# skhu101/TDNN-F_NAS

Hardware: AMD Instinct MI355X
Metric: LF-MMI training frames/sec per node (SWBD 7q TDNN-F) (higher is better)
Workload: dtype f32

## Files before the change

tdnn-f_nas_amd/csrc/abi_tdnn.hip:

```cpp
#include <dlfcn.h>
#include <stdlib.h>
#include <string.h>

#include <string>

#include "common.h"
#include "gemm_f32.h"
#include "planes_gemm.h"

namespace tdnnf {

static thread_local std::string g_last_error;

void set_error(const char *fmt, ...) {
  char buf[1024];
  va_list ap;
  va_start(ap, fmt);
  vsnprintf(buf, sizeof(buf), fmt, ap);
  va_end(ap);
  g_last_error = buf;
}
int hip_status(hipError_t e, const char *what) {
  set_error("HIP error %d (%s) in %s", (int)e, hipGetErrorString(e), what);
  return TDNNF_EHIP;
// ... 4 lines not shown
  return o;
}

namespace {
typedef int (*roctx_push_t)(const char *);
typedef int (*roctx_pop_t)();
roctx_push_t g_roctx_push = nullptr;
roctx_pop_t g_roctx_pop = nullptr;
bool roctx_ready() {
  static const bool ok = [] {
    const char *e = getenv("TDNNF_ROCTX");
    if (e && atoi(e) == 0) return false;
    for (const char *lib : {"librocprofiler-sdk-roctx.so", "librocprofiler-sdk-roctx.so.1", "libroctx64.so", "libroctx64.so.4"}) {
      void *h = dlopen(lib, RTLD_NOW | RTLD_GLOBAL);
      if (!h) continue;
      g_roctx_push = (roctx_push_t)dlsym(h, "roctxRangePushA");
      g_roctx_pop = (roctx_pop_t)dlsym(h, "roctxRangePop");
      if (g_roctx_push && g_roctx_pop) return true;
    }
    return false;
  }();
  return ok;
}
}
TraceRange::TraceRange(const char *name) : on(roctx_ready()) {
  if (on) g_roctx_push(name);
}
TraceRange::~TraceRange() {
  if (on) g_roctx_pop();
}

bool tdnn_rows_ok(const tdnnf_tdnn_indexes *ix, int rows_in, int N) {
  if (!ix || ix->num_offsets < 1 || ix->num_offsets > TDNNF_MAX_OFFSETS || ix->row_stride < 1) return false;
  for (int i = 0; i < ix->num_offsets; i++) {
    const long long need = (long long)ix->row_offsets[i] + (long long)ix->row_stride * N - (ix->row_stride - 1);
    if (ix->row_offsets[i] < 0 || (N > 0 && rows_in < need)) return false;
  }
  return true;
}

}

using namespace tdnnf;

extern "C" {

const char *tdnnf_last_error(void) { return g_last_error.c_str(); }
int tdnnf_abi_version(void) { return 1; }

static int *option_slot(const char *name) {
  Options &o = options();
  if (!name) return nullptr;
  const struct { const char *n; int *p; } table[] = {{"ng_grouped", &o.ng_grouped}, {"ng_fuse", &o.ng_fuse}, {"ng_early_in", &o.ng_early_in},
                                                     {"wgrad_stream", &o.wgrad_stream}, {"gemm_ring", &o.gemm_ring}, {"planes", &o.planes}, {"den_split", &o.den_split}, {"phase_events", &o.phase_events}, {"wgrad_lag", &o.wgrad_lag}, {"ng_bk", &o.ng_bk}, {"ng_valu", &o.ng_valu}, {"ng_pform", &o.ng_pform}, {"planes_group", &o.planes_group}, {"xent_behind_den", &o.xent_behind_den}, {"ng_early_fork", &o.ng_early_fork}, {"ng_diag_skip", &o.ng_diag_skip}, {"wgrad_small", &o.wgrad_small}, {"splitk_per_cu", &o.splitk_per_cu}, {"gemm_alt_taps", &o.gemm_alt_taps}, {"reverse_passes", &o.reverse_passes}, {"splitk_partial_round", &o.splitk_partial_round}, {"wgrad_on_caller", &o.wgrad_on_caller}, {"den_mw_test_abort", &o.den_mw_test_abort}, {"planes_check_bound", &o.planes_check_bound}, {"den_gamma_pairs", &o.den_gamma_pairs}, {"num_form", &o.num_form}, {"num_frontier_cap", &o.num_frontier_cap}, {"gemm_arith_test", &o.gemm_arith_test}};
  for (auto &e : table)
    if (strcmp(e.n, name) == 0) return e.p;
  return nullptr;
}
int tdnnf_set_option(const char *name, int value) {
  int *p = option_slot(name);
  TDNNF_REQUIRE(p, "set_option: unknown option '%s' (ng_grouped, ng_fuse, ng_early_in, wgrad_stream, gemm_ring, planes, den_split)", name ? name : "(null)");
  *p = value;
  return TDNNF_OK;
}
int tdnnf_get_option(const char *name, int *value) {
  int *p = option_slot(name);
  TDNNF_REQUIRE(p && value, "get_option: unknown option '%s'", name ? name : "(null)");
  *value = *p;
  return TDNNF_OK;
}

}

namespace tdnnf {
int tdnn_propagate_impl(const tdnnf_tdnn_indexes *ix, const tdnnf_mat *in, const float *W, int ldw, int Do, int Di,
                        const float *bias, const float *eff_coef, int init_mode, int relu, tdnnf_mat *out, tdnnf_stream stream,
                        float *colstats, int *colstats_rows) {
  TDNNF_REQUIRE(mat_ok(in) && mat_ok(out) && W, "tdnn_propagate: bad matrices");
  TDNNF_REQUIRE(Do > 0 && Di > 0 && in->cols == Di && out->cols == Do, "tdnn_propagate: dims: in.cols=%d Di=%d out.cols=%d Do=%d",
                in ? in->cols : -1, Di, out ? out->cols : -1, Do);
  TDNNF_REQUIRE(tdnn_rows_ok(ix, in->rows, out->rows), "tdnn_propagate: input has too few rows for the time offsets");
  TDNNF_REQUIRE(ldw >= ix->num_offsets * Di, "tdnn_propagate: ldw < K*Di");
  TDNNF_REQUIRE(init_mode >= 0 && init_mode <= 2 && (init_mode != 1 || bias), "tdnn_propagate: init_mode 1 needs a bias");
  RowsGemmArgs a;
  memset(&a, 0, sizeof(a));
  a.A = in->data;
  a.lda = (long long)in->stride * ix->row_stride;
  a.B = W;
  a.ldb = ldw;
  a.C = out->data;
  a.ldc = out->stride;
  a.M = out->rows;
  a.N = Do;
  a.bias = bias;
  a.coef = eff_coef;
  a.init_mode = init_mode;
  a.relu = relu;
  a.colstats = colstats;
  a.colstats_rows = colstats_rows;
  a.nseg = ix->num_offsets;
  for (int i = 0; i < a.nseg; i++) {
    a.seg[i].a_off = (long long)ix->row_offsets[i] * in->stride;
    a.seg[i].b_off = (long long)i * Di;
    a.seg[i].klen = Di;
    a.seg[i].m_lo = 0;
    a.seg[i].m_hi = out->rows;
  }
// ... 201 lines not shown
```

tdnn-f_nas_amd/csrc/common.h:

```cpp
#pragma once
#include <hip/hip_runtime.h>
#include <stdarg.h>
#include <stdio.h>

#include "tdnnf_hip.h"

namespace tdnnf {

struct MatView {
  float *data;
  int rows, cols, stride;
};
inline MatView view(const tdnnf_mat *m) { return MatView{m->data, m->rows, m->cols, m->stride}; }

void set_error(const char *fmt, ...);
int hip_status(hipError_t e, const char *what);

inline bool mat_ok(const tdnnf_mat *m) {
  return m && m->rows >= 0 && m->cols >= 0 && m->stride >= m->cols && (m->data || m->rows * m->cols == 0);
}
inline bool same_dim(const tdnnf_mat *a, const tdnnf_mat *b) { return a->rows == b->rows && a->cols == b->cols; }

inline bool vec4_ok(const MatView &m) {
  return (reinterpret_cast<uintptr_t>(m.data) & 15) == 0 && m.stride % 4 == 0 && m.cols % 4 == 0;
}

#define TDNNF_REQUIRE(cond, ...)            \
  do {                                      \
    if (!(cond)) {                          \
      ::tdnnf::set_error(__VA_ARGS__);      \
      return TDNNF_EINVAL;                  \
    }                                       \
  } while (0)

#define TDNNF_HIP(expr)                                         \
  do {                                                          \
    hipError_t e__ = (expr);                                    \
    if (e__ != hipSuccess) return ::tdnnf::hip_status(e__, #expr); \
  } while (0)

#define TDNNF_LAUNCH_CHECK() TDNNF_HIP(hipGetLastError())

struct Options {
  int ng_grouped = 1;
  int ng_fuse = 1;
  int ng_early_in = 1;
  int wgrad_stream = -1;
  int gemm_ring = 1;
  int planes = 1;
  int den_mw_test_abort = 0;
  int planes_group = 1;
  int planes_check_bound = 0;
  int wgrad_lag = 3;
  int wgrad_on_caller = 0;
  int splitk_partial_round = 1;
  int reverse_passes = 0;
  int gemm_alt_taps = 1;
  int splitk_per_cu = 2;
  int wgrad_small = 0;
  int ng_bk = 0;
  int ng_early_fork = 1;
  int xent_behind_den = -1;
  int ng_pform = 1;
  int ng_valu = 0;
  int ng_diag_skip = 0;
  int phase_events = 0;
  int den_split = -1;
  int num_form = 0;
  int gemm_arith_test = 0;
  int num_frontier_cap = 0;
  int den_gamma_pairs = 0;
};
Options &options();

struct TraceRange {
  explicit TraceRange(const char *name);
  ~TraceRange();
  bool on;
};

__host__ __device__ inline float floor_keep_nan(float x, float f) { return x < f ? f : x; }

inline int grid_for(long long work, int block, int cap = 2048) {
  long long g = (work + block - 1) / block;
  if (g > cap) g = cap;
  if (g < 1) g = 1;
  return (int)g;
}
#ifdef __HIPCC__
template <class T>
struct as_given { typedef T type; };
template <class... P>
__attribute__((visibility("hidden"))) inline hipError_t launch_vec_or_scalar(bool vec, int rows, int cols, void (*k4)(P...), void (*k1)(P...), hipStream_t s, typename as_given<P>::type... args) {
  const long long work = (long long)rows * (vec ? cols / 4 : cols);
  void (*k)(P...) = vec ? k4 : k1;
  hipLaunchKernelGGL(k, dim3(grid_for(work, 256)), dim3(256), 0, s, args...);
  return hipGetLastError();
}
#endif

inline unsigned long long tdnnf_decision(unsigned long long step, unsigned long long k) {
  unsigned long long z = step * 0x9E3779B97F4A7C15ULL + k * 0xBF58476D1CE4E5B9ULL + 0x94D049BB133111EBULL;
  z = (z ^ (z >> 30)) * 0xBF58476D1CE4E5B9ULL;
  z = (z ^ (z >> 27)) * 0x94D049BB133111EBULL;
  return (z ^ (z >> 31)) >> 8;
}

bool log_softmax_propagate_with_aux(const tdnnf_mat *in, tdnnf_mat *out, tdnnf_mat *aux, float aux_scale, hipStream_t s);
float chain_supervision_weight(const tdnnf_supervision *sp);
size_t chain_split_region_bytes(const tdnnf_den_graph *g, int B, int T);
int chain_den(const tdnnf_den_graph *g, const tdnnf_supervision *sp, const tdnnf_mat *y, float leaky, tdnnf_mat *deriv, void *ws, hipStream_t s,
              bool beside_other_work = false, hipStream_t caller_aux = nullptr, hipEvent_t ev_recursions = nullptr, bool *ev_recorded = nullptr);
int chain_num_recursion(const tdnnf_supervision *sp, const tdnnf_den_graph *g, const tdnnf_mat *y, void *ws, hipStream_t s);
int chain_num_xent(const tdnnf_den_graph *g, const tdnnf_supervision *sp, const tdnnf_mat *y, const tdnnf_mat *xent_output, float xent_regularize,
                   tdnnf_mat *xent_deriv, void *ws, hipStream_t s, bool xent_deriv_initialised = false);
int chain_num(const tdnnf_den_graph *g, const tdnnf_supervision *sp, const tdnnf_mat *y, const tdnnf_mat *xent_output,
              float xent_regularize, tdnnf_mat *xent_deriv, void *ws, hipStream_t s, bool xent_deriv_initialised = false);
int chain_finish(const tdnnf_den_graph *g, const tdnnf_supervision *sp, const tdnnf_mat *y, float l2_regularize, double *results,
                 tdnnf_mat *deriv, tdnnf_mat *xent_deriv, void *ws, hipStream_t s);
int chain_objf_den(const tdnnf_den_graph *g, const tdnnf_supervision *sp, const tdnnf_mat *y, float leaky, void *ws, hipStream_t s);
int chain_objf_num_recursion(const tdnnf_supervision *sp, const tdnnf_den_graph *g, const tdnnf_mat *y, void *ws, hipStream_t s);
int chain_objf_num_xent(const tdnnf_den_graph *g, const tdnnf_supervision *sp, const tdnnf_mat *y, const tdnnf_mat *xent_output, void *ws, hipStream_t s);
int chain_objf_finish(const tdnnf_den_graph *g, const tdnnf_supervision *sp, const tdnnf_mat *y, float l2_regularize, double *results, void *ws, hipStream_t s);
// ... 14 lines not shown
```

tdnn-f_nas_amd/csrc/launch_forms.h:

```cpp
#pragma once
#include <atomic>

namespace tdnnf {

enum RowsForm {
  kFormPlain,
  kFormRing,
  kFormSplitK,
  kFormPartialS2,
  kFormPartialS8 = kFormPartialS2 + 6,
  kFormMainSplitTail,
  kFormMainPlainTail,
  kFormSumsqPlain,
  kFormSumsqSplitK,
  kFormPost,
  kFormGrouped,
  kRowsForms
};
constexpr int kRowsTiles = 9, kRowsAriths = 3;

template <int WM, int WN, int TM, int TN, int BK>
constexpr int rows_tile_index() {
  constexpr int BM = WM * TM * 32, BN = WN * TN * 32;
  constexpr int t = (BM == 128 && BN == 32 && BK == 32) ? 0 : (BM == 128 && BN == 32 && BK == 64) ? 1 : (BM == 128 && BN == 64 && BK == 32) ? 2
                  : (BM == 128 && BN == 96 && BK == 16) ? 3 : (BM == 128 && BN == 96 && BK == 32) ? 4 : (BM == 128 && BN == 160 && BK == 16) ? 5
                  : (BM == 64 && BN == 128 && BK == 16) ? 6 : (BM == 128 && BN == 128 && BK == 16) ? 7 : (BM == 128 && BN == 128 && BK == 32) ? 8 : -1;
  static_assert(t >= 0, "a rows GEMM tile without a counter: add it here and to kRowsTileNames (launch_forms.hip)");
  return t;
}
constexpr int rows_form_index(int tile, int arith, int form) { return (tile * kRowsAriths + arith) * kRowsForms + form; }

enum {
  kPlanesPlain = kRowsTiles * kRowsAriths * kRowsForms,
  kPlanesMainSplitTail,
  kPlanesMainPlainTail,
  kWgradFirst,
  kWgradPlanes = kWgradFirst + 5 * kRowsAriths,
  kWgradLastSlabs,
  kRowsLastSlices,
  kRowsVec4Launches,
  kRowsScalarLaunches,
  kPlanesAltChunked,
  kLaunchFormCounters
};

std::atomic<long long> *launch_form_counters();
inline void count_form(int index) { launch_form_counters()[index].fetch_add(1, std::memory_order_relaxed); }
inline void note_rows_slices(int ksplit) { launch_form_counters()[kRowsLastSlices].store(ksplit, std::memory_order_relaxed); }
inline void note_wgrad_slabs(int splits) { launch_form_counters()[kWgradLastSlabs].store(splits, std::memory_order_relaxed); }

}
```

tdnn-f_nas_amd/csrc/launch_forms.hip:

```cpp
#include "launch_forms.h"

#include <stdio.h>

#include "common.h"

namespace tdnnf {

std::atomic<long long> *launch_form_counters() {
  static std::atomic<long long> counters[kLaunchFormCounters];
  return counters;
}

namespace {
const char *const kRowsTileNames[kRowsTiles] = {"128x32k32", "128x32k64", "128x64k32", "128x96k16", "128x96k32", "128x160k16", "64x128k16", "128x128k16", "128x128k32"};
const char *const kArithNames[kRowsAriths] = {"f32", "bf16x3", "bf16x6"};
const char *const kRowsFormNames[kRowsForms] = {"plain", "ring", "splitk", "partial_s2", "partial_s3", "partial_s4", "partial_s5", "partial_s6", "partial_s7", "partial_s8",
                                                "main_split_tail", "main_plain_tail", "sumsq_plain", "sumsq_splitk", "post", "grouped"};
const char *const kWgradTileNames[5] = {"128x128", "160x128", "128x160", "32x128", "64x64"};
}

}

using namespace tdnnf;

extern "C" {

const char *tdnnf_gemm_launch_form_name(int index) {
  static thread_local char buf[64];
  if (index < 0 || index >= kLaunchFormCounters) return nullptr;
  if (index < kPlanesPlain) {
    const int form = index % kRowsForms, arith = (index / kRowsForms) % kRowsAriths, tile = index / (kRowsForms * kRowsAriths);
    snprintf(buf, sizeof(buf), "rows.%s.%s.%s", kRowsTileNames[tile], kArithNames[arith], kRowsFormNames[form]);
  } else if (index == kPlanesPlain) {
    snprintf(buf, sizeof(buf), "planes.plain");
  } else if (index == kPlanesMainSplitTail) {
    snprintf(buf, sizeof(buf), "planes.main_split_tail");
  } else if (index == kPlanesMainPlainTail) {
    snprintf(buf, sizeof(buf), "planes.main_plain_tail");
  } else if (index < kWgradPlanes) {
    const int i = index - kWgradFirst;
    snprintf(buf, sizeof(buf), "wgrad.%s.%s", kWgradTileNames[i / kRowsAriths], kArithNames[i % kRowsAriths]);
  } else if (index == kWgradPlanes) {
    snprintf(buf, sizeof(buf), "wgrad.planes");
  } else if (index == kWgradLastSlabs) {
    snprintf(buf, sizeof(buf), "wgrad.last_slabs");
  } else if (index == kRowsLastSlices) {
    snprintf(buf, sizeof(buf), "rows.last_slices");
  } else if (index == kRowsVec4Launches) {
    snprintf(buf, sizeof(buf), "rows.launches_vec4");
  } else if (index == kRowsScalarLaunches) {
    snprintf(buf, sizeof(buf), "rows.launches_scalar");
  } else {
    snprintf(buf, sizeof(buf), "planes.alt_chunked");
  }
  return buf;
}

int tdnnf_gemm_launch_forms(long long *counts, int capacity, int reset) {
  std::atomic<long long> *c = launch_form_counters();
  for (int i = 0; i < kLaunchFormCounters; i++) {
    if (counts && i < capacity) counts[i] = c[i].load(std::memory_order_relaxed);
    if (reset) c[i].store(0, std::memory_order_relaxed);
  }
  return kLaunchFormCounters;
}

}
```

tdnn-f_nas_amd/csrc/ng_stats.hip:

```cpp
#include <string.h>

#include <algorithm>

#include "gemm_f32.h"
#include "ng.h"
#include "ng_kernels.h"

namespace tdnnf {
namespace {

size_t part_bytes(int N) { return ((size_t)rows_gemm_sumsq_blocks(N) * sizeof(double) + 63) & ~(size_t)63; }
size_t stats_ws_bytes(int Rp, int Di, int K, int N) {
  return part_bytes(N) + std::max(std::max(wgrad_workspace_bytes(Rp, Rp, 1, N), wgrad_workspace_bytes(Rp, Di, K, N)), ng_pform_ws_bytes(Rp, Di, K, N));
}

constexpr int kPformSpanCap = 4096;
struct TapSpan {
  int lo, hi;
};
TapSpan tap_span(const tdnnf_tdnn_indexes &ix) {
  TapSpan t{ix.row_offsets[0], ix.row_offsets[0]};
  for (int i = 1; i < ix.num_offsets; i++) {
    t.lo = std::min(t.lo, ix.row_offsets[i]);
    t.hi = std::max(t.hi, ix.row_offsets[i]);
// ... 26 lines not shown
  for (int i = 0; i < K; i++) tp.o[i] = in.ix.row_offsets[i] - sp.lo;
  const int M = N + (sp.hi - sp.lo);
  float *WP = (float *)ws;
  float *P = WP + (((size_t)K * Rp * Di + 63) & ~(size_t)63);
  double *psum = (double *)(P + (((size_t)M * K * Rp + 63) & ~(size_t)63));
  hipLaunchKernelGGL(stack_taps_kernel, dim3(grid_for((long long)K * Rp * Di, 256)), dim3(256), 0, s, W, Rp, ldw, Di, K, WP);
  TDNNF_HIP(rows_gemm_1seg(in.x.data + (size_t)sp.lo * in.x.stride, in.x.stride, WP, Di, true, P, K * Rp, M, K * Rp, Di, 2, nullptr, psum, s));
  hipLaunchKernelGGL(pform_combine_kernel, dim3(N / 128), dim3(256), 0, s, P, K * Rp, tp, Rp, bias, H, N, psum, part,
                     rows_gemm_sumsq_blocks(N));
  TDNNF_HIP(hipGetLastError());
  return TDNNF_OK;
}

RowsGemmArgs ng_pass_gemm_args(const float *W, int ldw, int Rp, const float *bias, const NgInput &in, float *H, int ldh, double *part) {
  const int N = in.N, K = in.ix.num_offsets, Di = in.Di;
  RowsGemmArgs a;
  memset(&a, 0, sizeof(a));
  a.A = in.x.data; a.lda = (long long)in.x.stride * in.ix.row_stride; a.B = W; a.ldb = ldw; a.C = H; a.ldc = ldh; a.M = N; a.N = Rp;
  a.bias = bias;
  a.init_mode = bias ? 1 : 2;
  a.coef = in.eff;
  a.sumsq = part;
  a.nseg = K;
  for (int i = 0; i < K; i++) {
    a.seg[i].a_off = (long long)in.ix.row_offsets[i] * in.x.stride;
    a.seg[i].b_off = (long long)i * Di;
    a.seg[i].klen = Di;
    a.seg[i].m_lo = 0;
    a.seg[i].m_hi = N;
  }
  return a;
}
NgRowdotArgs ng_pass_rowdot_args(const float *WT, int Rp, const float *bias, const NgInput &in, float *H, int ldh, double *part, int part_cap) {
  const int K = in.ix.num_offsets;
  NgRowdotArgs v;
  memset(&v, 0, sizeof(v));
  v.X = in.x.data; v.ldx = in.x.stride; v.row_stride = in.ix.row_stride; v.nseg = K; v.Di = in.Di; v.eff = in.eff; v.WT = WT; v.Rp = Rp;
  v.bias = bias; v.H = H; v.ldh = ldh; v.N = in.N; v.part = part; v.part_cap = part_cap;
  for (int i = 0; i < K; i++) v.seg_off[i] = (long long)in.ix.row_offsets[i] * in.x.stride;
  return v;
}

namespace {

const float *ones_column(const tdnnf_ng *ng, const NgInput &in) { return in.ones ? ng->wlast : nullptr; }

int stats_after_h(tdnnf_ng *ng, const NgInput &in, const float *H, void *wg_ws, size_t wg_bytes, bool upd, hipStream_t s) {
  const int N = in.N, K = in.ix.num_offsets, Di = in.Di, Rp = ng->Rp, Dp = ng->Dp, D = ng->D;
  ng->cur_upd = upd;
  ng->cur_N = N;
  ng->cur_ones = in.ones;
  if (!upd) return TDNNF_OK;
  TDNNF_REQUIRE(wg_ws && wg_bytes >= wgrad_workspace_bytes(Rp, Di, K, N), "ng: workspace too small");
  TDNNF_HIP(hipMemsetAsync(ng->J, 0, sizeof(float) * (size_t)Rp * Dp, s));
  if (in.ones) TDNNF_HIP(hipMemsetAsync(ng->tmpR, 0, sizeof(float) * Rp, s));
  WgradArgs j;
  memset(&j, 0, sizeof(j));
  j.dY = H; j.lddy = Rp; j.X = in.x.data; j.ldx = in.x.stride; j.Do = Rp; j.Di = Di; j.K = K; j.N = N; j.row_stride = in.ix.row_stride;
  for (int i = 0; i < K; i++) j.row_offsets[i] = in.ix.row_offsets[i];
  j.coef = in.eff; j.scale = 1.f; j.G = ng->J; j.ldg = Dp; j.accumulate = 1; j.bias_acc = in.ones ? ng->tmpR : nullptr;
  j.active = in.active; j.max_active = in.max_active;
  TDNNF_HIP(wgrad(j, wg_ws, wg_bytes, s));
  if (in.ones) hipLaunchKernelGGL(scatter_col_kernel, dim3((Rp + 63) / 64), dim3(64), 0, s, ng->tmpR, Rp, ng->J, Dp, D - 1);
  return TDNNF_OK;
}

int stats_main(tdnnf_ng *ng, const NgInput &in, float *H, double *part, void *wg_ws, size_t wg_bytes, bool upd, hipStream_t s) {
  const int N = in.N, K = in.ix.num_offsets, Di = in.Di, Rp = ng->Rp, Dp = ng->Dp;
  const float *bias = ones_column(ng, in);
  const NgRowdotArgs v = ng_pass_rowdot_args(ng->WT, Rp, bias, in, H, Rp, part, rows_gemm_sumsq_blocks(N));
  const int skip = options().ng_diag_skip;
  if (skip && ng->D != 0 && (((skip & 1) && K == 2 && Di >= 1024) || ((skip & 2) && !(K == 2 && Di >= 1024)))) {
    TDNNF_HIP(hipMemsetAsync(H, 0, sizeof(float) * (size_t)N * Rp, s));
    TDNNF_HIP(hipMemsetAsync(part, 0, sizeof(double) * rows_gemm_sumsq_blocks(N), s));
  } else if (ng_pform_ok(Rp, in, wg_bytes)) {
    int rc = ng_pform_pass(ng->W, Rp, Dp, bias, in, H, part, wg_ws, s);
    if (rc) return rc;
  } else if (options().ng_valu && !in.active && ng_rowdot_ok(v)) {
    TDNNF_HIP(ng_rowdot(v, s));
  } else {
    TDNNF_HIP(rows_gemm(ng_pass_gemm_args(ng->W, Dp, Rp, bias, in, H, Rp, part), true, s));
  }
  return stats_after_h(ng, in, H, wg_ws, wg_bytes, upd, s);
}

int stats_side(tdnnf_ng *ng, const float *H, const double *part, void *wg_ws, size_t wg_bytes, hipStream_t s) {
  const int N = ng->cur_N, Rp = ng->Rp, Dp = ng->Dp;
  TDNNF_REQUIRE(wg_ws && wg_bytes >= wgrad_workspace_bytes(Rp, Rp, 1, N), "ng: workspace too small");
  WgradArgs w;
  memset(&w, 0, sizeof(w));
  w.dY = H; w.lddy = Rp; w.X = H; w.ldx = Rp; w.Do = Rp; w.Di = Rp; w.K = 1; w.N = N; w.row_stride = 1; w.scale = 1.f;
  w.G = ng->Ld; w.ldg = Rp; w.accumulate = 0;
  TDNNF_HIP(wgrad(w, wg_ws, wg_bytes, s));
  hipLaunchKernelGGL(ng_scalars_kernel, dim3(1), dim3(256), 0, s, part, rows_gemm_sumsq_blocks(N), ng->cur_ones ? (double)N : 0.0, ng->Ld, ng->WWT,
                     Rp, ng->scal, ng->scale_f);
  if (!ng->cur_upd) return TDNNF_OK;
  TDNNF_HIP(rows_gemm_1seg(ng->J, Dp, ng->J, Dp, true, ng->Kd, Rp, Rp, Rp, Dp, 2, nullptr, nullptr, s));
  const size_t fRR = (size_t)Rp * Rp;
  TDNNF_HIP(hipMemcpyAsync(ng->h_K, ng->Kd, sizeof(float) * fRR, hipMemcpyDeviceToHost, s));
  TDNNF_HIP(hipMemcpyAsync(ng->h_L, ng->Ld, sizeof(float) * fRR, hipMemcpyDeviceToHost, s));
  TDNNF_HIP(hipMemcpyAsync(ng->h_tr0, ng->scal, sizeof(double), hipMemcpyDeviceToHost, s));
  TDNNF_HIP(hipEventRecord(ng->ev_job, s));
  ng_refresh_submit(ng, N, ng->ev_job);
  return TDNNF_OK;
}

int stats_core(tdnnf_ng *ng, const NgInput &in, float *H, void *ws, size_t ws_bytes, bool upd, hipStream_t s) {
  TDNNF_REQUIRE(ws && ws_bytes >= stats_ws_bytes(ng->Rp, in.Di, in.ix.num_offsets, in.N), "ng: workspace too small");
  double *part = (double *)ws;
  void *wg_ws = (char *)ws + part_bytes(in.N);
  const size_t wg_bytes = ws_bytes - part_bytes(in.N);
  int rc = stats_main(ng, in, H, part, wg_ws, wg_bytes, upd, s);
  if (rc) return rc;
// ... 147 lines not shown
```

tdnn-f_nas_amd/csrc/wgrad.hip:

```cpp
#include <algorithm>
#include <cstring>

#include "colreduce.h"
#include "common.h"
#include "device.h"
#include "gemm_f32.h"
#include "launch_forms.h"
#include "planes_gemm.h"
#include "wgrad_kernels.h"

namespace tdnnf {
namespace {

struct WgradPlan {
  int splits, rows_per_split, chunks, rows_per_chunk;
  size_t slab_floats, colsum_floats;
};

struct WgradTile {
  int BM, BN, variant;
};
inline int waste_of(int n, int t) { return ((n + t - 1) / t) * t - n; }
WgradTile wgrad_tile(int Do, int Di, bool x3 = false, int N = 1 << 30) {
  if (Do <= 32) return {32, 128, 3};
  if (!x3 && options().wgrad_small && N <= options().wgrad_small) return {64, 64, 4};
  if (x3) return {128, 128, 0};
  if (waste_of(Do, 160) * 128 < waste_of(Do, 128) * 160 && waste_of(Do, 160) < waste_of(Do, 128)) return {160, 128, 1};
  if (waste_of(Di, 160) < waste_of(Di, 128)) return {128, 160, 2};
  return {128, 128, 0};
}

constexpr size_t wgrad_lds_bytes(int BM, int BN) { return sizeof(float) * 2 * (32 * (BM + 4) + 32 * (BN + 4)); }
template <int NP>
constexpr size_t wgrad_x3_lds_bytes(int BM, int BN) {
  return sizeof(__bf16) * 2 * NP * (size_t)(BM + BN) * (NP == 2 ? 40 : 24);
}

template <int WM, int WN, int TM, int TN>
int wgrad_slots_of() {
  static int slots = 0;
  if (slots == 0) {
    int occ = 2;
    const int cus = device_cus();
    constexpr size_t lds = wgrad_lds_bytes(WM * TM * 32, WN * TN * 32);
    opt_in_lds(wgrad_kernel<WM, WN, TM, TN, 4>, lds);
    opt_in_lds(wgrad_kernel<WM, WN, TM, TN, 1>, lds);
    if (hipOccupancyMaxActiveBlocksPerMultiprocessor(&occ, (const void *)wgrad_kernel<WM, WN, TM, TN, 4>, 256, lds) != hipSuccess || occ < 1) occ = 2;
    slots = std::min(occ * cus, 1024);
    (void)hipGetLastError();
  }
  return slots;
}
int wgrad_slots(int variant) {
  if (variant == 4) return wgrad_slots_of<2, 2, 1, 1>();
  return variant == 1 ? wgrad_slots_of<1, 4, 5, 1>() : variant == 2 ? wgrad_slots_of<4, 1, 1, 5>() : variant == 3 ? wgrad_slots_of<1, 4, 1, 1>()
                                                                                                   : wgrad_slots_of<2, 2, 2, 2>();
}

inline int wgrad_min_rounds() { return 2; }

WgradPlan wgrad_plan(int Do, int Di, int K, int N, int slots, int ktaps = 0, bool x3 = false) {
  if (ktaps > 0) { WgradPlan p2 = wgrad_plan(Do, Di, ktaps, N, slots, 0, x3); p2.slab_floats = (size_t)p2.splits * Do * K * Di; return p2; }
  WgradPlan pl;
  const WgradTile wt = wgrad_tile(Do, Di, x3, N);
  const int tiles = ((Do + wt.BM - 1) / wt.BM) * K * ((Di + wt.BN - 1) / wt.BN);
  const int max_splits = std::max(1, (N + 255) / 256);
  int splits = 1;
  const int min_rounds = wgrad_min_rounds();
  for (int rounds = min_rounds; rounds <= std::max(4, min_rounds); rounds++) {
    splits = (rounds * slots) / tiles;
    if (splits >= 1 && (rounds * slots) / tiles * tiles >= rounds * slots * 3 / 4) break;
  }
  if (wt.variant == 4) splits = std::max(1, (2 * device_cus()) / tiles);
  if (splits < 1) splits = 1;
  if (splits > max_splits) splits = max_splits;
  int rps = (N + splits - 1) / splits;
  rps = ((rps + 31) / 32) * 32;
  pl.splits = (N + rps - 1) / rps;
  pl.rows_per_split = rps;
  pl.slab_floats = (size_t)pl.splits * Do * K * Di;
  pl.rows_per_chunk = 512;
  pl.chunks = (N + 511) / 512;
  pl.colsum_floats = (size_t)pl.chunks * Do;
  return pl;
}

struct WgradLaunch {
  dim3 grid;
  int ntm, ntn, rows_per_split;
  float *partial;
  hipStream_t s;
};
template <int WM, int WN, int TM, int TN, int TAG>
void launch_wgrad_tagged(const WgradLaunch &l, const WgradArgs &a_x, bool vec) {
  constexpr size_t lds = wgrad_lds_bytes(WM * TM * 32, WN * TN * 32);
  static const bool opted = opt_in_lds(wgrad_kernel<WM, WN, TM, TN, 4, TAG>, lds) && opt_in_lds(wgrad_kernel<WM, WN, TM, TN, 1, TAG>, lds);
  (void)opted;
  if (vec) hipLaunchKernelGGL((wgrad_kernel<WM, WN, TM, TN, 4, TAG>), l.grid, dim3(256), lds, l.s, a_x, l.ntm, l.ntn, l.rows_per_split, l.partial);
  else hipLaunchKernelGGL((wgrad_kernel<WM, WN, TM, TN, 1, TAG>), l.grid, dim3(256), lds, l.s, a_x, l.ntm, l.ntn, l.rows_per_split, l.partial);
}
template <int WM, int WN, int TM, int TN, int NP, int TAG>
void launch_wgrad_x3_tagged(const WgradLaunch &l, const WgradArgs &a) {
  constexpr size_t lds = wgrad_x3_lds_bytes<NP>(WM * TM * 32, WN * TN * 32);
  static const bool opted = opt_in_lds(wgrad_x3_kernel<WM, WN, TM, TN, NP, 1, TAG>, lds);
  (void)opted;
  hipLaunchKernelGGL((wgrad_x3_kernel<WM, WN, TM, TN, NP, 1, TAG>), l.grid, dim3(256), lds, l.s, a, l.ntm, l.ntn, l.rows_per_split, l.partial);
}
template <int WM, int WN, int TM, int TN, bool X3>
void launch_wgrad(const WgradLaunch &l, const WgradArgs &a, const WgradArgs &a_x, bool vec, int planes) {
  const bool ng = prof_class_override() == 3;
  if constexpr (X3) {
    if (planes == 2) {
      if (ng) launch_wgrad_x3_tagged<WM, WN, TM, TN, 2, 1>(l, a);
      else launch_wgrad_x3_tagged<WM, WN, TM, TN, 2, 0>(l, a);
      return;
    }
    if (planes == 3) {
      if (ng) launch_wgrad_x3_tagged<WM, WN, TM, TN, 3, 1>(l, a);
      else launch_wgrad_x3_tagged<WM, WN, TM, TN, 3, 0>(l, a);
      return;
    }
  }
  if (ng) launch_wgrad_tagged<WM, WN, TM, TN, 1>(l, a_x, vec);
  else launch_wgrad_tagged<WM, WN, TM, TN, 0>(l, a_x, vec);
}

hipError_t wgrad_finish(const WgradArgs &a, const float *partial, int splits, float *cs_partial, const float *ds1, const float *ds2, hipStream_t s) {
  hipError_t e;
  const long long total = (long long)a.Do * a.K * a.Di;
  int rb = (int)((total + 255) / 256);
  if (rb > 2048) rb = 2048;
  if (total <= 32768 && splits >= 8 && !ds1)
    hipLaunchKernelGGL(wgrad_reduce_small_kernel, dim3((unsigned)((total + 15) / 16)), dim3(256), 0, s, partial, splits, a.Do, a.K * a.Di,
                       a.Di, a.coef, a.scale, a.G, a.ldg, a.accumulate);
  else
    hipLaunchKernelGGL(wgrad_reduce_kernel, dim3(rb), dim3(256), 0, s, partial, splits, a.Do, a.K * a.Di, a.Di, a.coef,
                       a.scale, a.G, a.ldg, a.accumulate, ds1, ds2);
  e = hipGetLastError();
  if (e != hipSuccess) return e;
  if (a.bias_acc) {
    MatView dyv{const_cast<float *>(a.dY), a.N, a.Do, (int)a.lddy};
    e = colsum_add(dyv, a.scale, a.bias_acc, cs_partial, s);
  }
  return e;
}

bool planes_try_wgrad(const WgradArgs &a, void *workspace, size_t workspace_bytes, int np, hipStream_t s, hipError_t *err) {
  const PlanesOperand *hy = planes_hint_a(), *hx = planes_hint_b();
  if (!hy || !hx || hy->np != np || hx->np != np) return false;
  if (a.row_stride != 1 || a.K > 16 || a.K < 1) return false;
  if (a.dY != hy->base || a.lddy != hy->ld || a.N != hy->rows || a.Do != hy->cols) return false;
  if (a.ldx != hx->ld || a.X < hx->base || (a.X - hx->base) % hx->ld != 0 || a.Di != hx->cols) return false;
  const long long xrow0 = (a.X - hx->base) / hx->ld;
  const int nkb = (a.N + 15) / 16;
  if (nkb < 16) return false;
  const bool normal = a.Do >= a.Di;
  const int M = normal ? a.Do : a.Di, Nn = normal ? a.Di : a.Do;
  const int BM = planes_gemm_tile_rows(Nn), BN = planes_gemm_tile_cols(Nn);
  const int ntm = (M + BM - 1) / BM, ntn = (Nn + BN - 1) / BN;
// ... 57 lines not shown
}

}

size_t wgrad_workspace_bytes(int Do, int Di, int K, int N) {
  const WgradTile wt0 = wgrad_tile(Do, Di, false), wt1 = wgrad_tile(Do, Di, true);
  const int tiles = std::min(((Do + wt0.BM - 1) / wt0.BM) * ((Di + wt0.BN - 1) / wt0.BN),
                             ((Do + wt1.BM - 1) / wt1.BM) * ((Di + wt1.BN - 1) / wt1.BN));
  size_t max_splits = std::max<size_t>(1, std::min<size_t>((N + 255) / 256, std::max<size_t>((size_t)std::max(wgrad_min_rounds(), 4) * 1024 / tiles + 1, 16)));
  return sizeof(float) * (max_splits * Do * K * Di) + colreduce_bytes(N, Do) + 64;
}

hipError_t wgrad(const WgradArgs &a, void *workspace, size_t workspace_bytes, hipStream_t s) {
  if (a.N <= 0 || a.Do <= 0 || a.Di <= 0) return hipSuccess;
  if (workspace_bytes < wgrad_workspace_bytes(a.Do, a.Di, a.K, a.N)) return hipErrorInvalidValue;
  int planes = 0;
  {
    int prec = a.prec;
    if (prec == 0) {
      prec = gemm_precision_default();
      if (prec == 0 && (options().gemm_arith_test == 1 || options().gemm_arith_test == 3)) prec = options().gemm_arith_test;
    }
    if (prec == 4 || (prec == 3 && options().planes)) {
      hipError_t pe = hipSuccess;
      if (planes_try_wgrad(a, workspace, workspace_bytes, prec == 4 ? 2 : 3, s, &pe)) return pe;
    }
    planes = prec == 1 ? 2 : prec == 3 ? 3 : 0;
  }
  const bool use_x3 = planes != 0;
  const WgradTile wt = wgrad_tile(a.Do, a.Di, use_x3, a.N);
  const int ktaps = a.active && a.max_active > 0 && a.max_active < a.K ? a.max_active : a.K;
  WgradArgs a_x = a;
  a_x.xcd_order = ktaps > 1 ? 1 : 0;
  WgradPlan pl = wgrad_plan(a.Do, a.Di, a.K, a.N, wgrad_slots(wt.variant), ktaps == a.K ? 0 : ktaps, use_x3);
  if (sizeof(float) * pl.slab_floats > workspace_bytes) return hipErrorInvalidValue;
  float *partial = reinterpret_cast<float *>(workspace);
  float *cs_partial = partial + pl.slab_floats;
  const bool vec = aligned16(a.dY) && aligned16(a.X) && a.lddy % 4 == 0 && a.ldx % 4 == 0;
  const int ntm = (a.Do + wt.BM - 1) / wt.BM, ntn = (a.Di + wt.BN - 1) / wt.BN;
  const WgradLaunch l{dim3(ntm * ktaps * ntn, pl.splits), ntm, ntn, pl.rows_per_split, partial, s};
  {
    ProfFlopsScale exact(ktaps != a.K ? 1.0 : prof_flops_scale());
    const double flops = 2.0 * a.N * a.Do * ktaps * a.Di;
    if (prof_on()) {
      int lo = a.row_offsets[0], hi = a.row_offsets[0];
      for (int i = 1; i < a.K; i++) {
        lo = std::min(lo, a.row_offsets[i]);
        hi = std::max(hi, a.row_offsets[i]);
      }
      prof_next_gemm(flops, 4.0 * ((double)a.N * a.Do + std::min((double)a.N * ktaps, (double)a.N * a.row_stride + (hi - lo)) * a.Di +
                                   (double)a.Do * ktaps * a.Di * (a.accumulate ? 2.0 : 1.0)));
    }
    ProfScope ps(2, flops, s);
    count_form(kWgradFirst + wt.variant * kRowsAriths + (planes == 2 ? 1 : planes == 3 ? 2 : 0));
    note_wgrad_slabs(pl.splits);
    if (wt.variant == 4) launch_wgrad<2, 2, 1, 1, false>(l, a, a_x, vec, planes);
    else if (wt.variant == 1) launch_wgrad<1, 4, 5, 1, false>(l, a, a_x, vec, planes);
    else if (wt.variant == 2) launch_wgrad<4, 1, 1, 5, false>(l, a, a_x, vec, planes);
    else if (wt.variant == 3) launch_wgrad<1, 4, 1, 1, true>(l, a, a_x, vec, planes);
    else launch_wgrad<2, 2, 2, 2, true>(l, a, a_x, vec, planes);
  }
  hipError_t e = hipGetLastError();
  if (e != hipSuccess) return e;
  return wgrad_finish(a, partial, pl.splits, cs_partial, nullptr, nullptr, s);
}

}
```

tdnn-f_nas_amd/csrc/wgrad_kernels.h:

```cpp
#pragma once
#include "common.h"
#include "gemm_dev.h"
#include "gemm_f32.h"

namespace tdnnf {
namespace {

template <int WM, int WN, int TM, int TN, int VEC, int TAG = 0>
__global__ __launch_bounds__(256) void wgrad_kernel(const WgradArgs p, int ntm, int ntn_tap, int rows_per_split,
                                                    float *partial) {
  constexpr int BK = 32;
  constexpr int BM = WM * TM * 32, BN = WN * TN * 32;
  constexpr int LDAS = BM + 4, LDBS = BN + 4;
  constexpr int A_TILE = BK * LDAS, B_TILE = BK * LDBS;
  constexpr int A_F4 = (BM * BK / 4 + 255) / 256, B_F4 = (BN * BK / 4 + 255) / 256;
  extern __shared__ __attribute__((aligned(16))) float smem[];
  float *As = smem, *Bs = smem + 2 * A_TILE;

  const int tiles = ntm * (int)gridDim.x / ntm;
  int bid = blockIdx.x, split = blockIdx.y;
  int tile_m, tile_n, tap;
  if (p.xcd_order) {
    const int nb = gridDim.x * gridDim.y, b = blockIdx.y * gridDim.x + blockIdx.x;
    const int q = nb / 8, r = nb % 8, xcd = b % 8, j = b / 8;
// ... 103 lines not shown
#pragma unroll
    for (int k2 = 0; k2 < BK / 2; k2++) {
      const int cur = k2 & 1, nxt = cur ^ 1;
      if (k2 + 1 < BK / 2) {
#pragma unroll
        for (int i = 0; i < TM; i++) a[nxt][i] = as[(2 * k2 + 2) * LDAS + i * 32];
#pragma unroll
        for (int i = 0; i < TN; i++) b[nxt][i] = bs[(2 * k2 + 2) * LDBS + i * 32];
      }
#pragma unroll
      for (int i = 0; i < TM; i++)
#pragma unroll
        for (int j = 0; j < TN; j++)
          acc[i][j] = __builtin_amdgcn_mfma_f32_32x32x2f32(a[cur][i], b[cur][j], acc[i][j], 0, 0, 0);
    }
  };

  float *P = partial + (long long)split * p.Do * (p.K * p.Di);
  if (cf == 0.f) return;
  if (r_begin >= r_end) {
    for (int e = t; e < BM * BN; e += 256) {
      const int m = m0 + e / BN, n = n0 + e % BN;
      if (m < p.Do && n < p.Di) P[(long long)m * (p.K * p.Di) + tap * p.Di + n] = 0.f;
    }
    return;
  }
  load_tile(r_begin);
  store_tile(0);
  __syncthreads();
  {
    int buf = 0;
    for (int r0 = r_begin;; r0 += BK) {
      const bool more = r0 + BK < r_end;
      if (more) load_tile(r0 + BK);
      compute(buf);
      if (!more) break;
      store_tile(buf ^ 1);
      __syncthreads();
      buf ^= 1;
    }
  }
#pragma unroll
  for (int i = 0; i < TM; i++)
#pragma unroll
    for (int j = 0; j < TN; j++) {
      const int n = n0 + (wn * TN + j) * 32 + li;
      if (n >= p.Di) continue;
#pragma unroll
      for (int r = 0; r < 16; r++) {
        const int m = m0 + (wm * TM + i) * 32 + (r & 3) + 8 * (r >> 2) + 4 * lh;
        if (m < p.Do) P[(long long)m * (p.K * p.Di) + tap * p.Di + n] = acc[i][j][r];
      }
    }
}

template <int WM, int WN, int TM, int TN, int NP, int D, int TAG = 0>
__global__ __launch_bounds__(256, 2) void wgrad_x3_kernel(const WgradArgs p, int ntm, int ntn_tap, int rows_per_split, float *partial) {
  constexpr int BK = NP == 2 ? 32 : 16, LDH = BK + 8;
  constexpr int BM = WM * TM * 32, BN = WN * TN * 32;
  constexpr int A_IT = (BM * BK / 8 + 255) / 256, B_IT = (BN * BK / 8 + 255) / 256;
  extern __shared__ __attribute__((aligned(16))) float smem[];
  __bf16 *As = reinterpret_cast<__bf16 *>(smem);
  __bf16 *Bs = As + 2 * NP * BM * LDH;

  int bid = blockIdx.x;
  const int tile_m = bid % ntm;
  int tap = (bid / ntm) / ntn_tap;
  const int tile_n = (bid / ntm) % ntn_tap;
  if (p.active) {
    if (tap >= p.active[0]) return;
    tap = p.active[1 + tap];
  }
  const int m0 = tile_m * BM, n0 = tile_n * BN;
  const int split = blockIdx.y;
  const int r_begin = split * rows_per_split;
  const int r_end = min(p.N, r_begin + rows_per_split);
  const int t = threadIdx.x, lane = t & 63, wave = t >> 6;
  const int wm = wave / WN, wn = wave % WN, li = lane & 31, lh = lane >> 5;

  f32x16 acc[TM][TN];
#pragma unroll
  for (int a = 0; a < TM; a++)
#pragma unroll
    for (int b = 0; b < TN; b++)
#pragma unroll
      for (int r = 0; r < 16; r++) acc[a][b][r] = 0.f;

  const float cf = p.coef ? p.coef[tap] : 1.f;
  const float *Xb = p.X + (long long)p.row_offsets[tap] * p.ldx;
  const long long xrow = (long long)p.row_stride * p.ldx;

  float ra[D][A_IT][8], rb[D][B_IT][8];
  const float *aptr[A_IT], *bptr[B_IT];
  long long astep[A_IT], bstep[B_IT];
  int akg[A_IT], bkg[B_IT];
  {
    const float *zero = reinterpret_cast<const float *>(&g_zero4);
#pragma unroll
    for (int j = 0; j < A_IT; j++) {
      const int item = t + 256 * j, col = item % BM, kg = item / BM;
      const bool v = (BM * BK / 8 % 256 == 0 || item < BM * BK / 8) && m0 + col < p.Do;
      akg[j] = kg;
      aptr[j] = v ? p.dY + (long long)(kg * 8) * p.lddy + m0 + col : zero;
      astep[j] = v ? p.lddy : 0;
    }
#pragma unroll
// ... 251 lines not shown
```

Measured before the change: 1.628 million.

## Add two-tap shared-X wgrad kernel, 96-row tile, and skip J memset

Adds a weight-gradient kernel for the small-Do, two-tap case. It loads each X row tile once into LDS and accumulates both taps from it with MFMA, instead of reading X separately per tap. It also adds a 96x128 tile variant for Do up to 96. In the natural-gradient stats path, when the J output is fully covered, J is written directly instead of being zeroed with a memset and then accumulated. These changes aim to cut redundant global reads of X and one memset/read-modify-write pass, at the cost of more LDS per block and extra code paths gated by the new ng_j_form option.

New measurement: 1.635 million, median of 6. About the same (+0.4%).

```diff
diff --git a/tdnn-f_nas_amd/csrc/abi_tdnn.hip b/tdnn-f_nas_amd/csrc/abi_tdnn.hip
--- a/tdnn-f_nas_amd/csrc/abi_tdnn.hip
+++ b/tdnn-f_nas_amd/csrc/abi_tdnn.hip
@@ -80,7 +80,7 @@
   Options &o = options();
   if (!name) return nullptr;
   const struct { const char *n; int *p; } table[] = {{"ng_grouped", &o.ng_grouped}, {"ng_fuse", &o.ng_fuse}, {"ng_early_in", &o.ng_early_in},
-                                                     {"wgrad_stream", &o.wgrad_stream}, {"gemm_ring", &o.gemm_ring}, {"planes", &o.planes}, {"den_split", &o.den_split}, {"phase_events", &o.phase_events}, {"wgrad_lag", &o.wgrad_lag}, {"ng_bk", &o.ng_bk}, {"ng_valu", &o.ng_valu}, {"ng_pform", &o.ng_pform}, {"planes_group", &o.planes_group}, {"xent_behind_den", &o.xent_behind_den}, {"ng_early_fork", &o.ng_early_fork}, {"ng_diag_skip", &o.ng_diag_skip}, {"wgrad_small", &o.wgrad_small}, {"splitk_per_cu", &o.splitk_per_cu}, {"gemm_alt_taps", &o.gemm_alt_taps}, {"reverse_passes", &o.reverse_passes}, {"splitk_partial_round", &o.splitk_partial_round}, {"wgrad_on_caller", &o.wgrad_on_caller}, {"den_mw_test_abort", &o.den_mw_test_abort}, {"planes_check_bound", &o.planes_check_bound}, {"den_gamma_pairs", &o.den_gamma_pairs}, {"num_form", &o.num_form}, {"num_frontier_cap", &o.num_frontier_cap}, {"gemm_arith_test", &o.gemm_arith_test}};
+                                                     {"wgrad_stream", &o.wgrad_stream}, {"gemm_ring", &o.gemm_ring}, {"planes", &o.planes}, {"den_split", &o.den_split}, {"phase_events", &o.phase_events}, {"wgrad_lag", &o.wgrad_lag}, {"ng_bk", &o.ng_bk}, {"ng_valu", &o.ng_valu}, {"ng_pform", &o.ng_pform}, {"planes_group", &o.planes_group}, {"xent_behind_den", &o.xent_behind_den}, {"ng_early_fork", &o.ng_early_fork}, {"ng_diag_skip", &o.ng_diag_skip}, {"wgrad_small", &o.wgrad_small}, {"splitk_per_cu", &o.splitk_per_cu}, {"gemm_alt_taps", &o.gemm_alt_taps}, {"reverse_passes", &o.reverse_passes}, {"splitk_partial_round", &o.splitk_partial_round}, {"wgrad_on_caller", &o.wgrad_on_caller}, {"den_mw_test_abort", &o.den_mw_test_abort}, {"planes_check_bound", &o.planes_check_bound}, {"den_gamma_pairs", &o.den_gamma_pairs}, {"ng_j_form", &o.ng_j_form}, {"num_form", &o.num_form}, {"num_frontier_cap", &o.num_frontier_cap}, {"gemm_arith_test", &o.gemm_arith_test}};
   for (auto &e : table)
     if (strcmp(e.n, name) == 0) return e.p;
   return nullptr;
diff --git a/tdnn-f_nas_amd/csrc/common.h b/tdnn-f_nas_amd/csrc/common.h
--- a/tdnn-f_nas_amd/csrc/common.h
+++ b/tdnn-f_nas_amd/csrc/common.h
@@ -69,6 +69,7 @@
   int num_form = 0;
   int gemm_arith_test = 0;
   int num_frontier_cap = 0;
+  int ng_j_form = 1;
   int den_gamma_pairs = 0;
 };
 Options &options();
diff --git a/tdnn-f_nas_amd/csrc/launch_forms.h b/tdnn-f_nas_amd/csrc/launch_forms.h
--- a/tdnn-f_nas_amd/csrc/launch_forms.h
+++ b/tdnn-f_nas_amd/csrc/launch_forms.h
@@ -35,7 +35,7 @@
   kPlanesMainSplitTail,
   kPlanesMainPlainTail,
   kWgradFirst,
-  kWgradPlanes = kWgradFirst + 5 * kRowsAriths,
+  kWgradPlanes = kWgradFirst + 7 * kRowsAriths,
   kWgradLastSlabs,
   kRowsLastSlices,
   kRowsVec4Launches,
diff --git a/tdnn-f_nas_amd/csrc/launch_forms.hip b/tdnn-f_nas_amd/csrc/launch_forms.hip
--- a/tdnn-f_nas_amd/csrc/launch_forms.hip
+++ b/tdnn-f_nas_amd/csrc/launch_forms.hip
@@ -16,7 +16,7 @@
 const char *const kArithNames[kRowsAriths] = {"f32", "bf16x3", "bf16x6"};
 const char *const kRowsFormNames[kRowsForms] = {"plain", "ring", "splitk", "partial_s2", "partial_s3", "partial_s4", "partial_s5", "partial_s6", "partial_s7", "partial_s8",
                                                 "main_split_tail", "main_plain_tail", "sumsq_plain", "sumsq_splitk", "post", "grouped"};
-const char *const kWgradTileNames[5] = {"128x128", "160x128", "128x160", "32x128", "64x64"};
+const char *const kWgradTileNames[7] = {"128x128", "160x128", "128x160", "32x128", "64x64", "96x128", "32x128x2taps"};
 }
 
 }
diff --git a/tdnn-f_nas_amd/csrc/ng_stats.hip b/tdnn-f_nas_amd/csrc/ng_stats.hip
--- a/tdnn-f_nas_amd/csrc/ng_stats.hip
+++ b/tdnn-f_nas_amd/csrc/ng_stats.hip
@@ -102,13 +102,14 @@
   ng->cur_ones = in.ones;
   if (!upd) return TDNNF_OK;
   TDNNF_REQUIRE(wg_ws && wg_bytes >= wgrad_workspace_bytes(Rp, Di, K, N), "ng: workspace too small");
-  TDNNF_HIP(hipMemsetAsync(ng->J, 0, sizeof(float) * (size_t)Rp * Dp, s));
+  const bool j_store = options().ng_j_form && !in.ones && K * Di == Dp && !in.eff && !in.active;
+  if (!j_store) TDNNF_HIP(hipMemsetAsync(ng->J, 0, sizeof(float) * (size_t)Rp * Dp, s));
   if (in.ones) TDNNF_HIP(hipMemsetAsync(ng->tmpR, 0, sizeof(float) * Rp, s));
   WgradArgs j;
   memset(&j, 0, sizeof(j));
   j.dY = H; j.lddy = Rp; j.X = in.x.data; j.ldx = in.x.stride; j.Do = Rp; j.Di = Di; j.K = K; j.N = N; j.row_stride = in.ix.row_stride;
   for (int i = 0; i < K; i++) j.row_offsets[i] = in.ix.row_offsets[i];
-  j.coef = in.eff; j.scale = 1.f; j.G = ng->J; j.ldg = Dp; j.accumulate = 1; j.bias_acc = in.ones ? ng->tmpR : nullptr;
+  j.coef = in.eff; j.scale = 1.f; j.G = ng->J; j.ldg = Dp; j.accumulate = j_store ? 0 : 1; j.bias_acc = in.ones ? ng->tmpR : nullptr;
   j.active = in.active; j.max_active = in.max_active;
   TDNNF_HIP(wgrad(j, wg_ws, wg_bytes, s));
   if (in.ones) hipLaunchKernelGGL(scatter_col_kernel, dim3((Rp + 63) / 64), dim3(64), 0, s, ng->tmpR, Rp, ng->J, Dp, D - 1);
diff --git a/tdnn-f_nas_amd/csrc/wgrad.hip b/tdnn-f_nas_amd/csrc/wgrad.hip
--- a/tdnn-f_nas_amd/csrc/wgrad.hip
+++ b/tdnn-f_nas_amd/csrc/wgrad.hip
@@ -20,6 +20,7 @@
 struct WgradTile {
   int BM, BN, variant;
 };
+constexpr int kWgradTwoTap = 6;
 inline int waste_of(int n, int t) { return ((n + t - 1) / t) * t - n; }
 WgradTile wgrad_tile(int Do, int Di, bool x3 = false, int N = 1 << 30) {
   if (Do <= 32) return {32, 128, 3};
@@ -27,10 +28,12 @@
   if (x3) return {128, 128, 0};
   if (waste_of(Do, 160) * 128 < waste_of(Do, 128) * 160 && waste_of(Do, 160) < waste_of(Do, 128)) return {160, 128, 1};
   if (waste_of(Di, 160) < waste_of(Di, 128)) return {128, 160, 2};
+  if (options().ng_j_form && Do <= 96) return {96, 128, 5};
   return {128, 128, 0};
 }
 
 constexpr size_t wgrad_lds_bytes(int BM, int BN) { return sizeof(float) * 2 * (32 * (BM + 4) + 32 * (BN + 4)); }
+constexpr size_t kWgradTwoTapLds = sizeof(float) * 2 * (2 * 32 * (32 + 4) + 32 * (128 + 4));
 template <int NP>
 constexpr size_t wgrad_x3_lds_bytes(int BM, int BN) {
   return sizeof(__bf16) * 2 * NP * (size_t)(BM + BN) * (NP == 2 ? 40 : 24);
@@ -53,6 +56,7 @@
 }
 int wgrad_slots(int variant) {
   if (variant == 4) return wgrad_slots_of<2, 2, 1, 1>();
+  if (variant == 5) return wgrad_slots_of<1, 4, 3, 1>();
   return variant == 1 ? wgrad_slots_of<1, 4, 5, 1>() : variant == 2 ? wgrad_slots_of<4, 1, 1, 5>() : variant == 3 ? wgrad_slots_of<1, 4, 1, 1>()
                                                                                                    : wgrad_slots_of<2, 2, 2, 2>();
 }
@@ -105,6 +109,17 @@
   static const bool opted = opt_in_lds(wgrad_x3_kernel<WM, WN, TM, TN, NP, 1, TAG>, lds);
   (void)opted;
   hipLaunchKernelGGL((wgrad_x3_kernel<WM, WN, TM, TN, NP, 1, TAG>), l.grid, dim3(256), lds, l.s, a, l.ntm, l.ntn, l.rows_per_split, l.partial);
+}
+template <int TAG>
+void launch_wgrad_two_tap_tagged(const WgradLaunch &l, const WgradArgs &a, int lo, bool vec) {
+  static const bool opted = opt_in_lds(wgrad_two_tap_kernel<4, TAG>, kWgradTwoTapLds) && opt_in_lds(wgrad_two_tap_kernel<1, TAG>, kWgradTwoTapLds);
+  (void)opted;
+  if (vec) hipLaunchKernelGGL((wgrad_two_tap_kernel<4, TAG>), l.grid, dim3(256), kWgradTwoTapLds, l.s, a, lo, l.rows_per_split, l.partial);
+  else hipLaunchKernelGGL((wgrad_two_tap_kernel<1, TAG>), l.grid, dim3(256), kWgradTwoTapLds, l.s, a, lo, l.rows_per_split, l.partial);
+}
+bool wgrad_two_tap_ok(const WgradArgs &a, int planes) {
+  return options().ng_j_form && planes == 0 && a.Do <= 32 && a.K == 2 && a.row_stride == 1 && !a.coef && !a.active && a.Di >= 1024 &&
+         (a.row_offsets[1] - a.row_offsets[0]) % 32 == 0;
 }
 template <int WM, int WN, int TM, int TN, bool X3>
 void launch_wgrad(const WgradLaunch &l, const WgradArgs &a, const WgradArgs &a_x, bool vec, int planes) {
@@ -268,9 +283,16 @@
                                    (double)a.Do * ktaps * a.Di * (a.accumulate ? 2.0 : 1.0)));
     }
     ProfScope ps(2, flops, s);
-    count_form(kWgradFirst + wt.variant * kRowsAriths + (planes == 2 ? 1 : planes == 3 ? 2 : 0));
+    const bool two_tap = wt.variant == 3 && wgrad_two_tap_ok(a, planes);
+    count_form(kWgradFirst + (two_tap ? kWgradTwoTap : wt.variant) * kRowsAriths + (planes == 2 ? 1 : planes == 3 ? 2 : 0));
     note_wgrad_slabs(pl.splits);
-    if (wt.variant == 4) launch_wgrad<2, 2, 1, 1, false>(l, a, a_x, vec, planes);
+    if (two_tap) {
+      const WgradLaunch l2{dim3(ntn, pl.splits), 1, ntn, pl.rows_per_split, partial, s};
+      const int lo = a.row_offsets[1] < a.row_offsets[0] ? 1 : 0;
+      if (prof_class_override() == 3) launch_wgrad_two_tap_tagged<1>(l2, a, lo, vec);
+      else launch_wgrad_two_tap_tagged<0>(l2, a, lo, vec);
+    } else if (wt.variant == 5) launch_wgrad<1, 4, 3, 1, false>(l, a, a_x, vec, planes);
+    else if (wt.variant == 4) launch_wgrad<2, 2, 1, 1, false>(l, a, a_x, vec, planes);
     else if (wt.variant == 1) launch_wgrad<1, 4, 5, 1, false>(l, a, a_x, vec, planes);
     else if (wt.variant == 2) launch_wgrad<4, 1, 1, 5, false>(l, a, a_x, vec, planes);
     else if (wt.variant == 3) launch_wgrad<1, 4, 1, 1, true>(l, a, a_x, vec, planes);
diff --git a/tdnn-f_nas_amd/csrc/wgrad_kernels.h b/tdnn-f_nas_amd/csrc/wgrad_kernels.h
--- a/tdnn-f_nas_amd/csrc/wgrad_kernels.h
+++ b/tdnn-f_nas_amd/csrc/wgrad_kernels.h
@@ -179,6 +179,130 @@
         if (m < p.Do) P[(long long)m * (p.K * p.Di) + tap * p.Di + n] = acc[i][j][r];
       }
     }
+}
+
+template <int VEC, int TAG = 0>
+__global__ __launch_bounds__(256) void wgrad_two_tap_kernel(const WgradArgs p, int lo, int rows_per_split, float *partial) {
+  constexpr int BK = 32, BM = 32, BN = 128;
+  constexpr int LDAS = BM + 4, LDBS = BN + 4;
+  constexpr int A_TILE = BK * LDAS, B_TILE = BK * LDBS, B_F4 = BN * BK / 4 / 256;
+  extern __shared__ __attribute__((aligned(16))) float smem[];
+  float *As = smem, *Bs = smem + 4 * A_TILE;
+
+  const int hi = lo ^ 1;
+  const int d = p.row_offsets[hi] - p.row_offsets[lo];
+  const int n0 = blockIdx.x * BN, split = blockIdx.y;
+  const int r_begin = split * rows_per_split;
+  const int r_end = min(p.N, r_begin + rows_per_split);
+  const int q_end = r_end + d;
+  const int t = threadIdx.x, lane = t & 63, wn = t >> 6, li = lane & 31, lh = lane >> 5;
+
+  f32x16 acc[2];
+#pragma unroll
+  for (int a = 0; a < 2; a++)
+#pragma unroll
+    for (int r = 0; r < 16; r++) acc[a][r] = 0.f;
+
+  const float *Xb = p.X + (long long)p.row_offsets[lo] * p.ldx;
+
+  float4 ra[2], rb[B_F4];
+  const bool fast_ok = VEC == 4 && p.Do % 4 == 0 && p.Di % 4 == 0;
+  const float *zero = reinterpret_cast<const float *>(&g_zero4);
+  const int akr = t / (BM / 4), am = (t % (BM / 4)) * 4;
+  const bool av = am < p.Do;
+  const float *aptr = av ? p.dY + (long long)akr * p.lddy + am : zero;
+  const long long astep = av ? p.lddy : 0;
+  const float *bptr[B_F4];
+  long long bstep[B_F4];
+#pragma unroll
+  for (int j = 0; j < B_F4; j++) {
+    const int idx = t + 256 * j, kr = idx / (BN / 4), n = n0 + (idx % (BN / 4)) * 4;
+    const bool v = n < p.Di;
+    bptr[j] = v ? Xb + (long long)kr * p.ldx + n : zero;
+    bstep[j] = v ? p.ldx : 0;
+  }
+  auto load_tile = [&](int q0) {
+    const bool lo_full = q0 + BK <= r_end, lo_none = q0 >= r_end;
+    const bool hi_none = q0 < r_begin + d || q0 >= q_end, hi_full = !hi_none && q0 + BK <= q_end;
+    if (fast_ok && (lo_full || lo_none) && (hi_full || hi_none) && (lo_full || hi_full)) {
+      ra[0] = *reinterpret_cast<const float4 *>(lo_full ? aptr + (long long)q0 * astep : zero);
+      ra[1] = *reinterpret_cast<const float4 *>(hi_full ? aptr + (long long)(q0 - d) * astep : zero);
+#pragma unroll
+      for (int j = 0; j < B_F4; j++) rb[j] = *reinterpret_cast<const float4 *>(bptr[j] + (long long)q0 * bstep[j]);
+      return;
+    }
+    {
+      const int q = q0 + akr, h = q - d;
+      const bool v0 = q < r_end, v1 = h >= r_begin && h < r_end;
+      ra[0] = ld4(p.dY + (long long)(v0 ? q : 0) * p.lddy + am, v0 && am < p.Do, v0 && am + 1 < p.Do, v0 && am + 2 < p.Do, v0 && am + 3 < p.Do, VEC == 4);
+      ra[1] = ld4(p.dY + (long long)(v1 ? h : 0) * p.lddy + am, v1 && am < p.Do, v1 && am + 1 < p.Do, v1 && am + 2 < p.Do, v1 && am + 3 < p.Do, VEC == 4);
+    }
+#pragma unroll
+    for (int j = 0; j < B_F4; j++) {
+      const int idx = t + 256 * j;
+      const int q = q0 + idx / (BN / 4), n = n0 + (idx % (BN / 4)) * 4;
+      const bool rv = q < r_end || (q >= r_begin + d && q < q_end);
+      rb[j] = ld4(Xb + (long long)(rv ? q : 0) * p.ldx + n, rv && n < p.Di, rv && n + 1 < p.Di, rv && n + 2 < p.Di, rv && n + 3 < p.Di, VEC == 4);
+    }
+  };
+  auto store_tile = [&](int buf) {
+    float *as = As + buf * 2 * A_TILE, *bs = Bs + buf * B_TILE;
+    *reinterpret_cast<float4 *>(as + akr * LDAS + am) = ra[0];
+    *reinterpret_cast<float4 *>(as + A_TILE + akr * LDAS + am) = ra[1];
+#pragma unroll
+    for (int j = 0; j < B_F4; j++) {
+      const int idx = t + 256 * j;
+      *reinterpret_cast<float4 *>(bs + (idx / (BN / 4)) * LDBS + (idx % (BN / 4)) * 4) = rb[j];
+    }
+  };
+  auto compute = [&](int buf) {
+    const float *as = As + buf * 2 * A_TILE + lh * LDAS + li;
+    const float *bs = Bs + buf * B_TILE + lh * LDBS + wn * 32 + li;
+    float a[2][2], b[2];
+    a[0][0] = as[0];
+    a[0][1] = as[A_TILE];
+    b[0] = bs[0];
+#pragma unroll
+    for (int k2 = 0; k2 < BK / 2; k2++) {
+      const int cur = k2 & 1, nxt = cur ^ 1;
+      if (k2 + 1 < BK / 2) {
+        a[nxt][0] = as[(2 * k2 + 2) * LDAS];
+        a[nxt][1] = as[A_TILE + (2 * k2 + 2) * LDAS];
+        b[nxt] = bs[(2 * k2 + 2) * LDBS];
+      }
+      acc[0] = __builtin_amdgcn_mfma_f32_32x32x2f32(a[cur][0], b[cur], acc[0], 0, 0, 0);
+      acc[1] = __builtin_amdgcn_mfma_f32_32x32x2f32(a[cur][1], b[cur], acc[1], 0, 0, 0);
+    }
+  };
+
+  if (r_begin >= r_end) return;
+  load_tile(r_begin);
+  store_tile(0);
+  __syncthreads();
+  {
+    int buf = 0;
+    for (int q0 = r_begin;; q0 += BK) {
+      const bool more = q0 + BK < q_end;
+      if (more) load_tile(q0 + BK);
+      compute(buf);
+      if (!more) break;
+      store_tile(buf ^ 1);
+      __syncthreads();
+      buf ^= 1;
+    }
+  }
+  float *P = partial + (long long)split * p.Do * (2 * p.Di);
+  const int n = n0 + wn * 32 + li;
+  if (n >= p.Di) return;
+#pragma unroll
+  for (int a = 0; a < 2; a++) {
+    const int tap = a == 0 ? lo : hi;
+#pragma unroll
+    for (int r = 0; r < 16; r++) {
+      const int m = (r & 3) + 8 * (r >> 2) + 4 * lh;
+      if (m < p.Do) P[(long long)m * (2 * p.Di) + tap * p.Di + n] = acc[a][r];
+    }
+  }
 }
 
 template <int WM, int WN, int TM, int TN, int NP, int D, int TAG = 0>
```
